# mdw771/adorym

Measured on AMD Instinct MI355X. Metric: probe-positions/sec (fwd+grad), 256^3 multislice ptycho, higher is better.
Workload: dtype f32

## Files before the change

adorym_amd/csrc/adm_object.hip:

```cpp
#include <hip/hip_runtime.h>
#include <cstdlib>
#include <cstring>
#include <hip/hip_fp16.h>
#include "adm_common.h"
#include "adm_optim.h"
#include "adm_ms_math.h"

namespace adm {

struct RotGeom {
    int Y, X, Z, Yp, Xp, pad_y0, pad_x0;
};

struct Bilin {
    int i00, i01, i10, i11;
    float w00, w01, w10, w11;
};

__device__ __forceinline__ Bilin make_bilin(const uint16_t* coords, int xr, int zr, int X, int Z) {
#pragma clang fp contract(off)
    Bilin b;
    if (coords == nullptr) {
        b.i00 = b.i01 = b.i10 = b.i11 = xr * Z + zr;
        b.w00 = 1.f; b.w01 = b.w10 = b.w11 = 0.f;
// ... 31 lines not shown
    const int ya = y_lo + blockIdx.z * y_chunk;
    const int yb = min(ya + y_chunk, y_hi);
    const size_t plane = (size_t)g.X * g.Z;
    for (int y = ya; y < yb; ++y) {
        const float2* o = obj + (size_t)y * plane;
        const float2 v00 = o[b.i00], v01 = o[b.i01], v10 = o[b.i10], v11 = o[b.i11];
        float2 r;
        r.x = v00.x * b.w00 + v01.x * b.w01 + v10.x * b.w10 + v11.x * b.w11;
        r.y = v00.y * b.w00 + v01.y * b.w01 + v10.y * b.w10 + v11.y * b.w11;
        const size_t o_rot = ((size_t)zr * g.Yp + g.pad_y0 + y) * g.Xp + g.pad_x0 + xr;
        if (rot) rot[o_rot] = r;
        if (trans) trans[o_rot] = slice_transmission(r, k1, sigma);
    }
}

__global__ __launch_bounds__(256) void rotate_fwd_stack_kernel(const float2* __restrict__ obj, const uint16_t* const* __restrict__ tables,
                                                               int Yb, float2* __restrict__ rot, float2* __restrict__ trans, float k1,
                                                               float sigma, RotGeom g, int y_chunk) {
    const int xr = blockIdx.x * 16 + (threadIdx.x & 15);
    const int zr = blockIdx.y * 16 + (threadIdx.x >> 4);
    if (xr >= g.X || zr >= g.Z) return;
    const int ya = blockIdx.z * y_chunk;
    const int r = ya / Yb;
    const Bilin b = make_bilin(tables[r], xr, zr, g.X, g.Z);
    const int yb = min(ya + y_chunk, g.Y);
    const size_t plane = (size_t)g.X * g.Z;
    for (int y = ya; y < yb; ++y) {
        const float2* o = obj + (size_t)(y - r * Yb) * plane;
        const float2 v00 = o[b.i00], v01 = o[b.i01], v10 = o[b.i10], v11 = o[b.i11];
        float2 q;
        q.x = v00.x * b.w00 + v01.x * b.w01 + v10.x * b.w10 + v11.x * b.w11;
        q.y = v00.y * b.w00 + v01.y * b.w01 + v10.y * b.w10 + v11.y * b.w11;
        const size_t o_rot = ((size_t)zr * g.Yp + g.pad_y0 + y) * g.Xp + g.pad_x0 + xr;
        if (rot) rot[o_rot] = q;
        if (trans) trans[o_rot] = slice_transmission(q, k1, sigma);
    }
}

__global__ __launch_bounds__(256) void identity_fwd_kernel(const float2* __restrict__ obj, float2* __restrict__ rot, float2* __restrict__ trans,
                                                           float k1, float sigma, RotGeom g, int y_lo, int y_hi) {
    const size_t n = (size_t)(y_hi - y_lo) * g.X * g.Z;
    for (size_t i = (size_t)blockIdx.x * blockDim.x + threadIdx.x; i < n; i += (size_t)gridDim.x * blockDim.x) {
        const int z = (int)(i % g.Z);
        const size_t yx = i / g.Z;
        const int x = (int)(yx % g.X), y = y_lo + (int)(yx / g.X);
        const float2 r = obj[((size_t)y * g.X + x) * g.Z + z];
        const size_t o_rot = ((size_t)z * g.Yp + g.pad_y0 + y) * g.Xp + g.pad_x0 + x;
        if (rot) rot[o_rot] = r;
        if (trans) trans[o_rot] = slice_transmission(r, k1, sigma);
    }
}
__global__ __launch_bounds__(256) void identity_adj_kernel(const float2* __restrict__ grot, float2* __restrict__ gobj, RotGeom g, int y_lo,
                                                           int y_hi) {
    const size_t n = (size_t)(y_hi - y_lo) * g.X * g.Z;
    for (size_t i = (size_t)blockIdx.x * blockDim.x + threadIdx.x; i < n; i += (size_t)gridDim.x * blockDim.x) {
        const int z = (int)(i % g.Z);
        const size_t yx = i / g.Z;
        const int x = (int)(yx % g.X), y = y_lo + (int)(yx / g.X);
        const float2 v = grot[((size_t)z * g.Yp + g.pad_y0 + y) * g.Xp + g.pad_x0 + x];
        float2* o = gobj + ((size_t)y * g.X + x) * g.Z + z;
        float2 c = *o;
        c.x += v.x;
        c.y += v.y;
        *o = c;
    }
}

__global__ __launch_bounds__(256) void transmission_kernel(const float2* __restrict__ rot, float2* __restrict__ trans, float k1,
                                                           float sigma, int Z, int Yp, int Xp, int row_lo, int row_hi) {
    const size_t per = (size_t)(row_hi - row_lo) * Xp;
    const size_t n = per * Z;
    for (size_t i = (size_t)blockIdx.x * blockDim.x + threadIdx.x; i < n; i += (size_t)gridDim.x * blockDim.x) {
        const size_t z = i / per, r = i - z * per;
        const size_t o = (z * Yp + row_lo) * Xp + r;
        trans[o] = rot ? slice_transmission(rot[o], k1, sigma) : make_float2(1.f, 0.f);
    }
}

__global__ __launch_bounds__(256) void rotate_adj_kernel(const float2* __restrict__ grot, const uint16_t* __restrict__ coords,
                                                         float* __restrict__ gobj, RotGeom g, int y_lo, int y_hi, int y_chunk) {
    const int xr = blockIdx.x * 16 + (threadIdx.x & 15);
    const int zr = blockIdx.y * 16 + (threadIdx.x >> 4);
    if (xr >= g.X || zr >= g.Z) return;
    const Bilin b = make_bilin(coords, xr, zr, g.X, g.Z);
    const int ya = y_lo + blockIdx.z * y_chunk;
    const int yb = min(ya + y_chunk, y_hi);
    const size_t plane = (size_t)g.X * g.Z;
    for (int y = ya; y < yb; ++y) {
        const float2 v = grot[((size_t)zr * g.Yp + g.pad_y0 + y) * g.Xp + g.pad_x0 + xr];
        float* o = gobj + 2 * (size_t)y * plane;
        if (b.w00 != 0.f) { atomicAdd(o + 2 * b.i00, v.x * b.w00); atomicAdd(o + 2 * b.i00 + 1, v.y * b.w00); }
        if (b.w01 != 0.f) { atomicAdd(o + 2 * b.i01, v.x * b.w01); atomicAdd(o + 2 * b.i01 + 1, v.y * b.w01); }
        if (b.w10 != 0.f) { atomicAdd(o + 2 * b.i10, v.x * b.w10); atomicAdd(o + 2 * b.i10 + 1, v.y * b.w10); }
        if (b.w11 != 0.f) { atomicAdd(o + 2 * b.i11, v.x * b.w11); atomicAdd(o + 2 * b.i11 + 1, v.y * b.w11); }
    }
}

template <bool ALONG_X>
__global__ __launch_bounds__(256) void rotate_adj_csr_kernel(const float2* __restrict__ grot, const int* __restrict__ ptr,
                                                             const int* __restrict__ src, const float* __restrict__ wgt,
                                                             float2* __restrict__ gobj, RotGeom g, int y_lo, int y_hi) {
    __shared__ float2 tile[4][16][17];
    const int lx = ALONG_X ? (threadIdx.x & 15) : (threadIdx.x >> 4);
    const int lz = ALONG_X ? (threadIdx.x >> 4) : (threadIdx.x & 15);
    const int x = blockIdx.x * 16 + lx, z = blockIdx.y * 16 + lz;
    const bool ok = (x < g.X) && (z < g.Z);
    const int t = ok ? x * g.Z + z : 0;
    const int beg = ok ? ptr[t] : 0, end = ok ? ptr[t + 1] : 0;
    const int y0 = y_lo + blockIdx.z * 4;
    const int ny = min(4, y_hi - y0);
    const size_t plane = (size_t)g.X * g.Z;
    float2 a[4];
#pragma unroll
    for (int i = 0; i < 4; ++i) a[i] = make_float2(0.f, 0.f);
    const size_t row = (size_t)(g.pad_y0 + y0) * g.Xp;
    if (ny == 4) {
        for (int j = beg; j < end; ++j) {
            const float w = wgt[j];
            const float2* q = grot + (size_t)src[j] + row;
            const float2 v0 = q[0], v1 = q[g.Xp], v2 = q[2 * (size_t)g.Xp], v3 = q[3 * (size_t)g.Xp];
            a[0].x += w * v0.x; a[0].y += w * v0.y;
            a[1].x += w * v1.x; a[1].y += w * v1.y;
            a[2].x += w * v2.x; a[2].y += w * v2.y;
            a[3].x += w * v3.x; a[3].y += w * v3.y;
        }
    } else {
        for (int j = beg; j < end; ++j) {
            const float w = wgt[j];
            const float2* q = grot + (size_t)src[j] + row;
#pragma unroll
            for (int i = 0; i < 4; ++i)
                if (i < ny) { const float2 v = q[(size_t)i * g.Xp]; a[i].x += w * v.x; a[i].y += w * v.y; }
        }
    }
    int wx = lx, wz = lz;
    if (ALONG_X) {
#pragma unroll
        for (int i = 0; i < 4; ++i) tile[i][lx][lz] = a[i];
        __syncthreads();
        wx = threadIdx.x >> 4; wz = threadIdx.x & 15;
#pragma unroll
        for (int i = 0; i < 4; ++i) a[i] = tile[i][wx][wz];
    }
    const int ox = blockIdx.x * 16 + wx, oz = blockIdx.y * 16 + wz;
    if (ox < g.X && oz < g.Z) {
        float2* o = gobj + (size_t)y0 * plane + (size_t)ox * g.Z + oz;
#pragma unroll
        for (int i = 0; i < 4; ++i)
            if (i < ny) { float2 c = o[(size_t)i * plane]; c.x += a[i].x; c.y += a[i].y; o[(size_t)i * plane] = c; }
    }
}

#define ADM_STAGE_MAX 1024
__global__ __launch_bounds__(256) void rotate_adj_staged_kernel(const float2* __restrict__ grot, const int* __restrict__ ptr,
                                                                const int* __restrict__ src, const unsigned short* __restrict__ lsrc,
                                                                const float* __restrict__ wgt,
                                                                const int4* __restrict__ boxes, float2* __restrict__ gobj, RotGeom g,
                                                                int y_lo, int y_hi) {
    __shared__ float2 stage[4 * ADM_STAGE_MAX];
    const int4 box = boxes[blockIdx.y * gridDim.x + blockIdx.x];
    const int y0 = y_lo + blockIdx.z * 4;
    const int ny = min(4, y_hi - y0);
    const int bw = box.z, bh = box.w, per = bw * bh;
    const size_t slice = (size_t)g.Yp * g.Xp;
    const size_t plane = (size_t)g.X * g.Z;
    const int lx = threadIdx.x >> 4, lz = threadIdx.x & 15;
    const int x = blockIdx.x * 16 + lx, z = blockIdx.y * 16 + lz;
    const bool ok = (x < g.X) && (z < g.Z);
    const int t = ok ? x * g.Z + z : 0;
    const int beg = ok ? ptr[t] : 0, end = ok ? ptr[t + 1] : 0;
    float2* o = gobj + (size_t)y0 * plane + (size_t)x * g.Z + z;
    if (bw == 0) {
        if (!ok) return;
        const size_t row = (size_t)(g.pad_y0 + y0) * g.Xp;
        float2 a[4];
#pragma unroll
        for (int i = 0; i < 4; ++i) a[i] = make_float2(0.f, 0.f);
        for (int j = beg; j < end; ++j) {
            const float w = wgt[j];
            const float2* q = grot + (size_t)src[j] + row;
#pragma unroll
            for (int i = 0; i < 4; ++i)
                if (i < ny) { const float2 v = q[(size_t)i * g.Xp]; a[i].x += w * v.x; a[i].y += w * v.y; }
        }
#pragma unroll
        for (int i = 0; i < 4; ++i)
            if (i < ny) { float2 c = o[(size_t)i * plane]; c.x += a[i].x; c.y += a[i].y; o[(size_t)i * plane] = c; }
        return;
    }
    if (per <= ADM_STAGE_MAX) {
        for (int idx = threadIdx.x; idx < 4 * per; idx += 256) {
            const int p = idx / per, rem = idx - p * per;
            const int zz = rem / bw, xx = rem - zz * bw;
            float2 v = make_float2(0.f, 0.f);
            if (p < ny) v = grot[(size_t)(box.y + zz) * slice + (size_t)(g.pad_y0 + y0 + p) * g.Xp + g.pad_x0 + box.x + xx];
            stage[p * ADM_STAGE_MAX + rem] = v;
        }
        __syncthreads();
        if (!ok) return;
        float2 a[4];
#pragma unroll
        for (int i = 0; i < 4; ++i) a[i] = make_float2(0.f, 0.f);
        for (int j = beg; j < end; ++j) {
            const float w = wgt[j];
            const int q = lsrc[j];
#pragma unroll
            for (int i = 0; i < 4; ++i) { const float2 v = stage[i * ADM_STAGE_MAX + q]; a[i].x += w * v.x; a[i].y += w * v.y; }
        }
#pragma unroll
        for (int i = 0; i < 4; ++i)
            if (i < ny) { float2 c = o[(size_t)i * plane]; c.x += a[i].x; c.y += a[i].y; o[(size_t)i * plane] = c; }
        return;
    }
    const int npp = (2 * per <= 4 * ADM_STAGE_MAX) ? 2 : 1;
    for (int p0 = 0; p0 < ny; p0 += npp) {
        for (int idx = threadIdx.x; idx < npp * per; idx += 256) {
            const int pp = idx / per, rem = idx - pp * per;
            const int zz = rem / bw, xx = rem - zz * bw;
            float2 v = make_float2(0.f, 0.f);
            if (p0 + pp < ny) v = grot[(size_t)(box.y + zz) * slice + (size_t)(g.pad_y0 + y0 + p0 + pp) * g.Xp + g.pad_x0 + box.x + xx];
            stage[idx] = v;
        }
        __syncthreads();
        if (ok) {
            float2 acc0 = make_float2(0.f, 0.f), acc1 = make_float2(0.f, 0.f);
            const int second = (npp == 2) ? per : 0;
            for (int j = beg; j < end; j += 8) {
                float w[8];
                int q[8];
#pragma unroll
                for (int u = 0; u < 8; ++u) {
                    const int jj = min(j + u, end - 1);
                    w[u] = (j + u < end) ? wgt[jj] : 0.f;
                    q[u] = lsrc[jj];
                }
#pragma unroll
                for (int u = 0; u < 8; ++u) {
                    const float2 v0 = stage[q[u]];
                    const float2 v1 = stage[q[u] + second];
                    acc0.x += w[u] * v0.x; acc0.y += w[u] * v0.y;
                    acc1.x += w[u] * v1.x; acc1.y += w[u] * v1.y;
                }
            }
            float2 c = o[(size_t)p0 * plane];
            c.x += acc0.x;
            c.y += acc0.y;
            o[(size_t)p0 * plane] = c;
            if (npp == 2 && p0 + 1 < ny) {
                float2 d = o[(size_t)(p0 + 1) * plane];
                d.x += acc1.x;
                d.y += acc1.y;
                o[(size_t)(p0 + 1) * plane] = d;
            }
        }
        __syncthreads();
    }
}

struct AdjTables { const int* ptr; const int* src; const unsigned short* lsrc; const float* wgt; const int4* boxes; };
__global__ __launch_bounds__(256) void rotate_adj_staged_stack_kernel(const float2* __restrict__ grot, const AdjTables* __restrict__ tabs,
                                                                      int R, int Yb, float2* __restrict__ gobj, RotGeom g, int npl,
                                                                      float2* __restrict__ part) {
    __shared__ float2 stage[4 * ADM_STAGE_MAX];
    const int nzg = (Yb + npl - 1) / npl;
    const int zg = part ? (int)blockIdx.z % nzg : (int)blockIdx.z;
    const int r_lo = part ? (int)blockIdx.z / nzg : 0, r_hi = part ? r_lo + 1 : R;
    const int y0 = zg * npl;
    const int ny = min(npl, Yb - y0);
    const size_t slice = (size_t)g.Yp * g.Xp;
    const size_t plane = (size_t)g.X * g.Z;
    const int lx = threadIdx.x >> 4, lz = threadIdx.x & 15;
    const int x = blockIdx.x * 16 + lx, z = blockIdx.y * 16 + lz;
    const bool ok = (x < g.X) && (z < g.Z);
    const int t = ok ? x * g.Z + z : 0;
    float2* o = (part ? part + (size_t)r_lo * Yb * plane : gobj) + (size_t)y0 * plane + (size_t)x * g.Z + z;
    float2 c[4];
#pragma unroll
    for (int i = 0; i < 4; ++i) c[i] = (ok && i < ny && !part) ? o[(size_t)i * plane] : make_float2(0.f, 0.f);
    for (int r = r_lo; r < r_hi; ++r) {
        const AdjTables T = tabs[r];
        const int4 box = T.boxes[blockIdx.y * gridDim.x + blockIdx.x];
        const int ys = r * Yb + y0;
        const int bw = box.z, bh = box.w, per = bw * bh;
        const int beg = ok ? T.ptr[t] : 0, end = ok ? T.ptr[t + 1] : 0;
        if (bw == 0) {
            const size_t row = (size_t)(g.pad_y0 + ys) * g.Xp;
            float2 a[4];
#pragma unroll
            for (int i = 0; i < 4; ++i) a[i] = make_float2(0.f, 0.f);
            for (int j = beg; j < end; ++j) {
                const float w = T.wgt[j];
                const float2* q = grot + (size_t)T.src[j] + row;
#pragma unroll
                for (int i = 0; i < 4; ++i)
                    if (i < ny) { const float2 v = q[(size_t)i * g.Xp]; a[i].x += w * v.x; a[i].y += w * v.y; }
            }
#pragma unroll
            for (int i = 0; i < 4; ++i) { c[i].x += a[i].x; c[i].y += a[i].y; }
        } else if (per <= ADM_STAGE_MAX) {
            for (int idx = threadIdx.x; idx < npl * per; idx += 256) {
                const int p = idx / per, rem = idx - p * per;
                const int zz = rem / bw, xx = rem - zz * bw;
                float2 v = make_float2(0.f, 0.f);
                if (p < ny) v = grot[(size_t)(box.y + zz) * slice + (size_t)(g.pad_y0 + ys + p) * g.Xp + g.pad_x0 + box.x + xx];
                stage[p * ADM_STAGE_MAX + rem] = v;
            }
            __syncthreads();
            float2 a[4];
#pragma unroll
            for (int i = 0; i < 4; ++i) a[i] = make_float2(0.f, 0.f);
            for (int j = beg; j < end; ++j) {
                const float w = T.wgt[j];
                const int q = T.lsrc[j];
#pragma unroll
                for (int i = 0; i < 4; ++i)
                    if (i < ny) { const float2 v = stage[i * ADM_STAGE_MAX + q]; a[i].x += w * v.x; a[i].y += w * v.y; }
            }
#pragma unroll
            for (int i = 0; i < 4; ++i) { c[i].x += a[i].x; c[i].y += a[i].y; }
        } else {
            const int npp = (npl >= 2 && 2 * per <= 4 * ADM_STAGE_MAX) ? 2 : 1;
            for (int p0 = 0; p0 < ny; p0 += npp) {
                for (int idx = threadIdx.x; idx < npp * per; idx += 256) {
                    const int pp = idx / per, rem = idx - pp * per;
                    const int zz = rem / bw, xx = rem - zz * bw;
                    float2 v = make_float2(0.f, 0.f);
                    if (p0 + pp < ny) v = grot[(size_t)(box.y + zz) * slice + (size_t)(g.pad_y0 + ys + p0 + pp) * g.Xp + g.pad_x0 + box.x + xx];
                    stage[idx] = v;
                }
                __syncthreads();
                float2 acc0 = make_float2(0.f, 0.f), acc1 = make_float2(0.f, 0.f);
                const int second = (npp == 2) ? per : 0;
                for (int j = beg; j < end; j += 8) {
                    float w[8];
                    int q[8];
#pragma unroll
                    for (int u = 0; u < 8; ++u) {
                        const int jj = min(j + u, end - 1);
                        w[u] = (j + u < end) ? T.wgt[jj] : 0.f;
                        q[u] = T.lsrc[jj];
                    }
#pragma unroll
                    for (int u = 0; u < 8; ++u) {
                        const float2 v0 = stage[q[u]];
                        const float2 v1 = stage[q[u] + second];
                        acc0.x += w[u] * v0.x; acc0.y += w[u] * v0.y;
                        acc1.x += w[u] * v1.x; acc1.y += w[u] * v1.y;
                    }
                }
#pragma unroll
                for (int i = 0; i < 4; ++i) {
                    if (i == p0) { c[i].x += acc0.x; c[i].y += acc0.y; }
                    if (npp == 2 && i == p0 + 1) { c[i].x += acc1.x; c[i].y += acc1.y; }
                }
                __syncthreads();
            }
        }
        __syncthreads();
    }
    if (ok) {
#pragma unroll
        for (int i = 0; i < 4; ++i)
            if (i < ny) o[(size_t)i * plane] = c[i];
    }
}

#define ADM_MAXCOVER 64

struct TileGeom {
    int Yp, Xp, pad_y0, pad_x0, Py, Px, R1, R2, G, LPW, NT, n_steps, binning, Z;
    int pixel_major;
    int row_elems;
    int row0, nrows;
    int add_lo, add_hi;
};

__global__ __launch_bounds__(256) void cover_build_kernel(const int2* __restrict__ pos, int b0, int B, TileGeom g,
                                                          unsigned* __restrict__ cover, int* __restrict__ overflow) {
    __shared__ int2 sp[256];
    __shared__ int sb[256];
    __shared__ int wcnt[4];
    const int x = blockIdx.x * 32 + (threadIdx.x & 31);
    const int r = blockIdx.y * 8 + (threadIdx.x >> 5);
    const bool live = x < g.Xp && r < g.nrows;
    const int y = g.row0 + r;
    const int bx_lo = blockIdx.x * 32, by_lo = g.row0 + blockIdx.y * 8;
    const size_t cplane = (size_t)g.nrows * g.Xp;
    unsigned* out = cover + (size_t)(live ? r : 0) * g.Xp + (live ? x : 0);
    int cnt = 0;
    const unsigned per_pos = (unsigned)g.n_steps * g.row_elems;
    const int wave = threadIdx.x >> 6, lane = threadIdx.x & 63;
    for (int c0 = b0; c0 < B; c0 += 256) {
        const int b = c0 + (int)threadIdx.x;
        int2 p = make_int2(0, 0);
        bool hit = false;
        if (b < B) {
            p = pos[b];
            const int ty = p.x + g.pad_y0, tx = p.y + g.pad_x0;
            hit = ty < by_lo + 8 && ty + g.Py > by_lo && tx < bx_lo + 32 && tx + g.Px > bx_lo;
        }
        const unsigned long long m = __ballot(hit);
        __syncthreads();
        if (lane == 0) wcnt[wave] = __popcll(m);
        __syncthreads();
        int off = 0, n = 0;
#pragma unroll
        for (int w = 0; w < 4; ++w) { if (w < wave) off += wcnt[w]; n += wcnt[w]; }
        if (hit) {
            const int k = off + __popcll(m & ((1ull << lane) - 1ull));
// ... 559 lines not shown
    if (reg_value) {
        __shared__ float red[4];
#pragma unroll
        for (int off = 32; off > 0; off >>= 1) val += __shfl_down(val, off, 64);
        if ((threadIdx.x & 63) == 0) red[threadIdx.x >> 6] = val;
        __syncthreads();
        if (threadIdx.x == 0) atomicAdd(reg_value, red[0] + red[1] + red[2] + red[3]);
    }
}

__global__ __launch_bounds__(256) void axpy_kernel(float* __restrict__ y, const float* __restrict__ x, float a, size_t n) {
    for (size_t i = (size_t)blockIdx.x * blockDim.x + threadIdx.x; i < n; i += (size_t)gridDim.x * blockDim.x)
        y[i] += a * x[i];
}

static inline int stream_grid(size_t n) {
    size_t b = (n + 255) / 256;
    return (int)(b > 4096 ? 4096 : (b ? b : 1));
}

}

using namespace adm;

extern "C" int adm_rotate_fwd(adm_plan* plan, const float* obj, const uint16_t* coords, float* obj_rot, int y_lo, int y_hi) {
    if (!plan || !obj || !obj_rot) return fail(ADM_ERR_INVALID, "adm_rotate_fwd: null argument");
    const adm_plan_desc& d = plan->d;
    if (y_lo < 0 || y_hi > d.obj_y || y_lo > y_hi) return fail(ADM_ERR_INVALID, "adm_rotate_fwd: bad y range");
    if (y_lo == y_hi) return ADM_OK;
    RotGeom g{d.obj_y, d.obj_x, d.obj_z, plan->Yp, plan->Xp, d.pad_y0, d.pad_x0};
    int y_chunk = 32;
    const int n_patch = ((d.obj_x + 15) / 16) * ((d.obj_z + 15) / 16);
    while (y_chunk > 1 && n_patch * ((y_hi - y_lo + y_chunk - 1) / y_chunk) < 512) y_chunk >>= 1;
    dim3 grid((d.obj_x + 15) / 16, (d.obj_z + 15) / 16, (y_hi - y_lo + y_chunk - 1) / y_chunk);
    float2* rot_out = (plan->trans_dev && plan->trans_only) ? (float2*)nullptr : (float2*)obj_rot;
    if (!coords && d.obj_z < 16)
        hipLaunchKernelGGL(identity_fwd_kernel, dim3(stream_grid((size_t)(y_hi - y_lo) * d.obj_x * d.obj_z)), dim3(256), 0, plan->ctx->stream,
                           (const float2*)obj, rot_out, plan->trans_dev, d.k1, (float)d.sign_convention, g, y_lo, y_hi);
    else
        hipLaunchKernelGGL(rotate_fwd_kernel, grid, dim3(256), 0, plan->ctx->stream, (const float2*)obj, coords, rot_out, plan->trans_dev,
                           d.k1, (float)d.sign_convention, g, y_lo, y_hi, y_chunk);
    ADM_HIP(hipGetLastError());
    if (plan->trans_dev) plan->trans_src = obj_rot;
    return ADM_OK;
}

extern "C" int adm_rotate_fwd_stack(adm_plan* plan, const float* obj, const void* tables_dev, int n_tables, float* obj_rot) {
    if (!plan || !obj || !tables_dev || !obj_rot) return fail(ADM_ERR_INVALID, "adm_rotate_fwd_stack: null argument");
    const adm_plan_desc& d = plan->d;
    if (n_tables < 1 || d.obj_y % n_tables) return fail(ADM_ERR_INVALID, "adm_rotate_fwd_stack: the plan's y extent is not n_tables blocks");
    const int Yb = d.obj_y / n_tables;
    RotGeom g{d.obj_y, d.obj_x, d.obj_z, plan->Yp, plan->Xp, d.pad_y0, d.pad_x0};
    int y_chunk = 32;
    while (y_chunk > 1 && Yb % y_chunk) y_chunk >>= 1;
    const int n_patch = ((d.obj_x + 15) / 16) * ((d.obj_z + 15) / 16);
    while (y_chunk > 1 && n_patch * (d.obj_y / y_chunk) < 512) y_chunk >>= 1;
    dim3 grid((d.obj_x + 15) / 16, (d.obj_z + 15) / 16, d.obj_y / y_chunk);
    float2* rot_out = (plan->trans_dev && plan->trans_only) ? (float2*)nullptr : (float2*)obj_rot;
    hipLaunchKernelGGL(rotate_fwd_stack_kernel, grid, dim3(256), 0, plan->ctx->stream, (const float2*)obj,
                       (const uint16_t* const*)tables_dev, Yb, rot_out, plan->trans_dev, d.k1, (float)d.sign_convention, g, y_chunk);
    ADM_HIP(hipGetLastError());
    if (plan->trans_dev) plan->trans_src = obj_rot;
    return ADM_OK;
}

static int transmission_fill(adm_plan* plan, const float* obj_rot, int row_lo, int row_hi) {
    const adm_plan_desc& d = plan->d;
    const size_t n = (size_t)(row_hi - row_lo) * plan->Xp * d.obj_z;
    hipLaunchKernelGGL(transmission_kernel, dim3((unsigned)std::min<size_t>((n + 255) / 256, 8192)), dim3(256), 0, plan->ctx->stream,
                       (const float2*)obj_rot, plan->trans_dev, d.k1, (float)d.sign_convention, d.obj_z, plan->Yp, plan->Xp, row_lo,
                       row_hi);
    ADM_HIP(hipGetLastError());
    return ADM_OK;
}

extern "C" int adm_plan_set_transmission_cache(adm_plan* plan, int on) {
    if (!plan) return fail(ADM_ERR_INVALID, "adm_plan_set_transmission_cache: null plan");
    const adm_plan_desc& d = plan->d;
    if (!on) {
        if (plan->trans_dev) {
            ADM_HIP(hipStreamSynchronize(plan->ctx->main_stream));
            ADM_HIP(hipFree(plan->trans_dev));
        }
        plan->trans_dev = nullptr;
        plan->trans_src = nullptr;
        plan->trans_only = false;
        return ADM_OK;
    }
    if (d.unknown_type != 0 || d.binning != 1)
        return fail(ADM_ERR_UNSUPPORTED, "adm_plan_set_transmission_cache: needs unknown_type delta_beta and binning 1");
    if (!plan->trans_dev) {
        float2* t = nullptr;
        ADM_HIP(hipMalloc((void**)&t, (size_t)d.obj_z * plan->Yp * plan->Xp * sizeof(float2)));
        plan->trans_dev = t;
        plan->trans_src = nullptr;
        const int rc = transmission_fill(plan, nullptr, 0, plan->Yp);
        if (rc) {
            (void)hipFree(t);
            plan->trans_dev = nullptr;
            plan->trans_only = false;
            return rc;
        }
    }
    plan->trans_only = (on == 2);
    return ADM_OK;
}

extern "C" int adm_transmission_refresh(adm_plan* plan, const float* obj_rot, int y_lo, int y_hi) {
    if (!plan || !obj_rot) return fail(ADM_ERR_INVALID, "adm_transmission_refresh: null argument");
    if (!plan->trans_dev) return fail(ADM_ERR_INVALID, "adm_transmission_refresh: the plan has no transmission cache");
    const adm_plan_desc& d = plan->d;
    if (y_lo < 0 || y_hi > d.obj_y || y_lo > y_hi) return fail(ADM_ERR_INVALID, "adm_transmission_refresh: bad y range");
    plan->trans_src = obj_rot;
    if (y_lo == y_hi) return ADM_OK;
    return transmission_fill(plan, obj_rot, d.pad_y0 + y_lo, d.pad_y0 + y_hi);
}

extern "C" int adm_rotate_adj(adm_plan* plan, const float* grad_rot, const uint16_t* coords, float* grad_obj, int y_lo, int y_hi) {
    if (!plan || !grad_rot || !grad_obj) return fail(ADM_ERR_INVALID, "adm_rotate_adj: null argument");
    const adm_plan_desc& d = plan->d;
    if (y_lo < 0 || y_hi > d.obj_y || y_lo > y_hi) return fail(ADM_ERR_INVALID, "adm_rotate_adj: bad y range");
    if (y_lo == y_hi) return ADM_OK;
    RotGeom g{d.obj_y, d.obj_x, d.obj_z, plan->Yp, plan->Xp, d.pad_y0, d.pad_x0};
    const int y_chunk = 32;
    dim3 grid((d.obj_x + 15) / 16, (d.obj_z + 15) / 16, (y_hi - y_lo + y_chunk - 1) / y_chunk);
    if (!coords && d.obj_z < 16)
        hipLaunchKernelGGL(identity_adj_kernel, dim3(stream_grid((size_t)(y_hi - y_lo) * d.obj_x * d.obj_z)), dim3(256), 0, plan->ctx->stream,
                           (const float2*)grad_rot, (float2*)grad_obj, g, y_lo, y_hi);
    else
        hipLaunchKernelGGL(rotate_adj_kernel, grid, dim3(256), 0, plan->ctx->stream, (const float2*)grad_rot, coords, grad_obj, g, y_lo,
                           y_hi, y_chunk);
    ADM_HIP(hipGetLastError());
    return ADM_OK;
}

extern "C" int adm_rotate_adj_csr(adm_plan* plan, const float* grad_rot, const int32_t* csr_ptr, const int32_t* csr_src,
                                  const float* csr_w, float* grad_obj, int y_lo, int y_hi, int lanes_along_x) {
    if (!plan || !grad_rot || !csr_ptr || !csr_src || !csr_w || !grad_obj) return fail(ADM_ERR_INVALID, "adm_rotate_adj_csr: null argument");
    const adm_plan_desc& d = plan->d;
    if (y_lo < 0 || y_hi > d.obj_y || y_lo > y_hi) return fail(ADM_ERR_INVALID, "adm_rotate_adj_csr: bad y range");
    if (y_lo == y_hi) return ADM_OK;
    RotGeom g{d.obj_y, d.obj_x, d.obj_z, plan->Yp, plan->Xp, d.pad_y0, d.pad_x0};
    dim3 grid((d.obj_x + 15) / 16, (d.obj_z + 15) / 16, (y_hi - y_lo + 3) / 4);
    if (lanes_along_x)
        hipLaunchKernelGGL(rotate_adj_csr_kernel<true>, grid, dim3(256), 0, plan->ctx->stream, (const float2*)grad_rot, csr_ptr, csr_src,
                           csr_w, (float2*)grad_obj, g, y_lo, y_hi);
    else
        hipLaunchKernelGGL(rotate_adj_csr_kernel<false>, grid, dim3(256), 0, plan->ctx->stream, (const float2*)grad_rot, csr_ptr, csr_src,
                           csr_w, (float2*)grad_obj, g, y_lo, y_hi);
    ADM_HIP(hipGetLastError());
    return ADM_OK;
}

extern "C" int adm_rotate_adj_staged(adm_plan* plan, const float* grad_rot, const int32_t* csr_ptr, const int32_t* csr_src,
                                     const uint16_t* csr_lsrc, const float* csr_w, const int32_t* boxes, float* grad_obj, int y_lo,
                                     int y_hi) {
    if (!plan || !grad_rot || !csr_ptr || !csr_src || !csr_lsrc || !csr_w || !boxes || !grad_obj)
        return fail(ADM_ERR_INVALID, "adm_rotate_adj_staged: null argument");
    const adm_plan_desc& d = plan->d;
    if (y_lo < 0 || y_hi > d.obj_y || y_lo > y_hi) return fail(ADM_ERR_INVALID, "adm_rotate_adj_staged: bad y range");
    if (y_lo == y_hi) return ADM_OK;
    RotGeom g{d.obj_y, d.obj_x, d.obj_z, plan->Yp, plan->Xp, d.pad_y0, d.pad_x0};
    dim3 grid((d.obj_x + 15) / 16, (d.obj_z + 15) / 16, (y_hi - y_lo + 3) / 4);
    hipLaunchKernelGGL(rotate_adj_staged_kernel, grid, dim3(256), 0, plan->ctx->stream, (const float2*)grad_rot, csr_ptr, csr_src,
                       (const unsigned short*)csr_lsrc, csr_w, (const int4*)boxes, (float2*)grad_obj, g, y_lo, y_hi);
    ADM_HIP(hipGetLastError());
    return ADM_OK;
}

#ifndef ADM_STACK_MIN_BLOCKS
#define ADM_STACK_MIN_BLOCKS 2048
#endif
__global__ __launch_bounds__(256) void stack_sum_kernel(const float2* __restrict__ part, int R, size_t n, float2* __restrict__ gobj) {
    const size_t i = (size_t)blockIdx.x * 256 + threadIdx.x;
    if (i >= n) return;
    float2 c = gobj[i];
    for (int r = 0; r < R; ++r) {
        const float2 a = part[(size_t)r * n + i];
        c.x += a.x;
        c.y += a.y;
    }
    gobj[i] = c;
}

extern "C" int adm_rotate_adj_staged_stack(adm_plan* plan, const float* grad_rot, const void* tables_dev, int n_tables, float* grad_obj,
                                           float* scratch, size_t scratch_bytes) {
    if (!plan || !grad_rot || !tables_dev || !grad_obj) return fail(ADM_ERR_INVALID, "adm_rotate_adj_staged_stack: null argument");
    const adm_plan_desc& d = plan->d;
    if (n_tables < 1 || d.obj_y % n_tables) return fail(ADM_ERR_INVALID, "adm_rotate_adj_staged_stack: the plan's y extent is not n_tables blocks");
    const int Yb = d.obj_y / n_tables;
    RotGeom g{d.obj_y, d.obj_x, d.obj_z, plan->Yp, plan->Xp, d.pad_y0, d.pad_x0};
    int npl = 4;
    const int n_patch = ((d.obj_x + 15) / 16) * ((d.obj_z + 15) / 16);
    while (npl > 1 && n_patch * ((Yb + npl - 1) / npl) < 1024) npl >>= 1;
    const size_t n_real = (size_t)Yb * d.obj_x * d.obj_z;
    if (scratch) {
        if (scratch_bytes < (size_t)n_tables * n_real * sizeof(float2))
            return fail(ADM_ERR_INVALID, "adm_rotate_adj_staged_stack: scratch smaller than n_tables x the real object");
        npl = 4;
        while (npl > 1 && (size_t)n_patch * ((Yb + npl - 1) / npl) * n_tables < (size_t)ADM_STACK_MIN_BLOCKS) npl >>= 1;
        dim3 gridp((d.obj_x + 15) / 16, (d.obj_z + 15) / 16, ((Yb + npl - 1) / npl) * n_tables);
        hipLaunchKernelGGL(rotate_adj_staged_stack_kernel, gridp, dim3(256), 0, plan->ctx->stream, (const float2*)grad_rot,
                           (const AdjTables*)tables_dev, n_tables, Yb, (float2*)grad_obj, g, npl, (float2*)scratch);
        hipLaunchKernelGGL(stack_sum_kernel, dim3((unsigned)((n_real + 255) / 256)), dim3(256), 0, plan->ctx->stream,
                           (const float2*)scratch, n_tables, n_real, (float2*)grad_obj);
        ADM_HIP(hipGetLastError());
        return ADM_OK;
    }
    dim3 grid((d.obj_x + 15) / 16, (d.obj_z + 15) / 16, (Yb + npl - 1) / npl);
    hipLaunchKernelGGL(rotate_adj_staged_stack_kernel, grid, dim3(256), 0, plan->ctx->stream, (const float2*)grad_rot,
                       (const AdjTables*)tables_dev, n_tables, Yb, (float2*)grad_obj, g, npl, (float2*)nullptr);
    ADM_HIP(hipGetLastError());
    return ADM_OK;
}

extern "C" int adm_tile_grad_accumulate(adm_plan* plan, void* workspace, size_t workspace_bytes, const int32_t* pos, int batch,
                                       const int32_t* pos_host, float* grad_rot) {
    return adm_tile_grad_accumulate_part(plan, workspace, workspace_bytes, pos, batch, pos_host, grad_rot, 0, 0, 0);
}

static int tile_geom(adm_plan* plan, int batch, const int32_t* pos_host, int win_y_lo, int win_y_hi, int add, TileGeom& g) {
    const adm_plan_desc& d = plan->d;
    const int N = d.probe_x;
    g.Yp = plan->Yp; g.Xp = plan->Xp; g.pad_y0 = d.pad_y0; g.pad_x0 = d.pad_x0; g.Py = d.probe_y; g.Px = d.probe_x;
    g.pixel_major = plan->generic ? 1 : 0;
    g.row_elems = (int)ms_row_elems(plan);
    g.R1 = g.R2 = g.G = g.LPW = 1; g.NT = 64;
    if (!plan->generic) { g.R1 = ms_r1_for(N); g.R2 = ms_r2_for(N); g.G = g.R1 > g.R2 ? g.R1 : g.R2; g.LPW = 64 / g.G; g.NT = ms_threads_for(N); }
    g.n_steps = plan->n_steps; g.binning = d.binning; g.Z = d.obj_z;
    int ymin = pos_host[0], ymax = pos_host[0];
    for (int b = 1; b < batch; ++b) { ymin = pos_host[2 * b] < ymin ? pos_host[2 * b] : ymin; ymax = pos_host[2 * b] > ymax ? pos_host[2 * b] : ymax; }
    g.row0 = ymin + d.pad_y0;
    g.nrows = ymax - ymin + d.probe_y;
    g.add_lo = g.add_hi = 0;
    if (add) {
        g.add_lo = g.row0;
        g.add_hi = g.row0 + g.nrows;
    } else if (win_y_hi > win_y_lo) {
        if (win_y_lo + d.pad_y0 > g.row0 || win_y_hi + d.pad_y0 < g.row0 + g.nrows)
            return fail(ADM_ERR_INVALID, "adm_tile_grad_accumulate_part: the window must contain the part's own rows");
        g.row0 = win_y_lo + d.pad_y0;
        g.nrows = win_y_hi - win_y_lo;
    }
    if (g.row0 < 0 || g.row0 + g.nrows > g.Yp) return fail(ADM_ERR_INVALID, "adm_tile_grad_accumulate: a position lies outside the padded frame");
    const size_t per = (size_t)plan->n_steps * g.row_elems;
    if ((size_t)batch * per >= 0xFFFFFFFFull) return fail(ADM_ERR_UNSUPPORTED, "adm_tile_grad_accumulate: batch too large for 32-bit tile offsets");
    return ADM_OK;
}

static unsigned long long pos_fingerprint(const int32_t* pos_host, int batch) {
    unsigned long long h = 1469598103934665603ull;
    for (int i = 0; i < 2 * batch; ++i) { h ^= (unsigned)pos_host[i]; h *= 1099511628211ull; }
    return h;
}
static void cover_key_put(adm_plan* plan, const void* ws, const void* pos, const int32_t* pos_host, int batch, const TileGeom& g) {
    int slot = 0;
    for (int i = 0; i < 4; ++i) {
        if (plan->cover_keys[i].ws == ws) { slot = i; break; }
        if (!plan->cover_keys[i].ws) slot = i;
    }
    plan->cover_keys[slot] = {ws, pos, batch, g.row0, g.nrows, pos_fingerprint(pos_host, batch)};
}
static bool cover_key_take(adm_plan* plan, const void* ws, const void* pos, const int32_t* pos_host, int batch, const TileGeom& g) {
    for (int i = 0; i < 4; ++i) {
        adm_plan::CoverKey& k = plan->cover_keys[i];
        if (k.ws == ws) {
            const bool ok = k.pos == pos && k.batch == batch && k.row0 == g.row0 && k.nrows == g.nrows && k.fp == pos_fingerprint(pos_host, batch);
            k.ws = nullptr;
            return ok;
        }
    }
    return false;
}

static int cover_build(adm_plan* plan, void* workspace, const int32_t* pos, int batch, const TileGeom& g, int b_lo = 0, int b_hi = -1) {
    if (b_hi < 0) b_hi = batch;
    char* ws = (char*)workspace;
    unsigned* cover = (unsigned*)(ws + ws_off_cover(plan, batch));
    int* overflow = (int*)(cover + (size_t)g.Yp * g.Xp * (ADM_MAXCOVER + 1));
    hipStream_t st = plan->ctx->stream;
    if (b_hi - b_lo > ADM_MAXCOVER) ADM_HIP(hipMemsetAsync(overflow, 0, sizeof(int), st));
    dim3 grid((g.Xp + 31) / 32, (g.nrows + 7) / 8, 1);
    hipLaunchKernelGGL(cover_build_kernel, grid, dim3(256), 0, st, (const int2*)pos, b_lo, b_hi, g, cover, overflow);
    ADM_HIP(hipGetLastError());
    return ADM_OK;
}

extern "C" int adm_tile_cover_build(adm_plan* plan, void* workspace, size_t workspace_bytes, const int32_t* pos, int batch,
                                    const int32_t* pos_host, int win_y_lo, int win_y_hi, int add) {
    if (!plan || !workspace || !pos || !pos_host) return fail(ADM_ERR_INVALID, "adm_tile_cover_build: null argument");
    if (batch <= 0) return fail(ADM_ERR_INVALID, "adm_tile_cover_build: batch must be positive");
    if (workspace_bytes < adm_plan_workspace_bytes(plan, batch)) return fail(ADM_ERR_INVALID, "adm_tile_cover_build: workspace too small");
    TileGeom g;
    int rc = tile_geom(plan, batch, pos_host, win_y_lo, win_y_hi, add, g);
    if (rc) return rc;
    rc = cover_build(plan, workspace, pos, batch, g);
    if (rc) return rc;
    cover_key_put(plan, workspace, pos, pos_host, batch, g);
    return ADM_OK;
}

extern "C" int adm_tile_grad_accumulate_part(adm_plan* plan, void* workspace, size_t workspace_bytes, const int32_t* pos, int batch,
                                            const int32_t* pos_host, float* grad_rot, int win_y_lo, int win_y_hi, int add) {
    if (!plan || !workspace || !pos || !pos_host || !grad_rot) return fail(ADM_ERR_INVALID, "adm_tile_grad_accumulate: null argument");
    if (batch <= 0) return fail(ADM_ERR_INVALID, "adm_tile_grad_accumulate: batch must be positive");
    if (workspace_bytes < adm_plan_workspace_bytes(plan, batch)) return fail(ADM_ERR_INVALID, "adm_tile_grad_accumulate: workspace too small");
    TileGeom g;
    int rc = tile_geom(plan, batch, pos_host, win_y_lo, win_y_hi, add, g);
    if (rc) return rc;
    const bool prebuilt = cover_key_take(plan, workspace, pos, pos_host, batch, g);
    if (!prebuilt) {
        rc = cover_build(plan, workspace, pos, batch, g);
        if (rc) return rc;
    }
    char* ws = (char*)workspace;
    const float2* gtile = (const float2*)(ws + ws_off_gtile(plan, batch));
    unsigned* cover = (unsigned*)(ws + ws_off_cover(plan, batch));
    hipStream_t st = plan->ctx->stream;
// ... 236 lines not shown
```

Before: 15110.

## Remap staged rotate-adjoint grid to 1D with per-plane border tiles and XCD-aware interior

The staged rotate-adjoint kernel now launches a flat 1D grid by default. Border-ring tiles that use the unstaged or large-box path are split into one block per y-plane to spread their heavier work, and interior tiles are distributed in contiguous chunks per XCD slot (block index mod 8) for better L2 locality across MI355X's chiplets. The old 3D grid remains available via ADM_ROT_XCD=0. The change adds index arithmetic and some early-exit padding blocks, and it assumes an 8-way round-robin dispatch of blocks to XCDs.

```diff
diff --git a/adorym_amd/csrc/adm_object.hip b/adorym_amd/csrc/adm_object.hip
--- a/adorym_amd/csrc/adm_object.hip
+++ b/adorym_amd/csrc/adm_object.hip
@@ -207,20 +207,15 @@
 }
 
 #define ADM_STAGE_MAX 1024
-__global__ __launch_bounds__(256) void rotate_adj_staged_kernel(const float2* __restrict__ grot, const int* __restrict__ ptr,
-                                                                const int* __restrict__ src, const unsigned short* __restrict__ lsrc,
-                                                                const float* __restrict__ wgt,
-                                                                const int4* __restrict__ boxes, float2* __restrict__ gobj, RotGeom g,
-                                                                int y_lo, int y_hi) {
-    __shared__ float2 stage[4 * ADM_STAGE_MAX];
-    const int4 box = boxes[blockIdx.y * gridDim.x + blockIdx.x];
-    const int y0 = y_lo + blockIdx.z * 4;
-    const int ny = min(4, y_hi - y0);
+__device__ __forceinline__ void adj_staged_planes(float2* __restrict__ stage, const float2* __restrict__ grot, const int* __restrict__ ptr,
+                                                  const int* __restrict__ src, const unsigned short* __restrict__ lsrc,
+                                                  const float* __restrict__ wgt, const int4 box, float2* __restrict__ gobj,
+                                                  const RotGeom& g, int bx, int bz, int y0, int ny) {
     const int bw = box.z, bh = box.w, per = bw * bh;
     const size_t slice = (size_t)g.Yp * g.Xp;
     const size_t plane = (size_t)g.X * g.Z;
     const int lx = threadIdx.x >> 4, lz = threadIdx.x & 15;
-    const int x = blockIdx.x * 16 + lx, z = blockIdx.y * 16 + lz;
+    const int x = bx * 16 + lx, z = bz * 16 + lz;
     const bool ok = (x < g.X) && (z < g.Z);
     const int t = ok ? x * g.Z + z : 0;
     const int beg = ok ? ptr[t] : 0, end = ok ? ptr[t + 1] : 0;
@@ -267,7 +262,7 @@
             if (i < ny) { float2 c = o[(size_t)i * plane]; c.x += a[i].x; c.y += a[i].y; o[(size_t)i * plane] = c; }
         return;
     }
-    const int npp = (2 * per <= 4 * ADM_STAGE_MAX) ? 2 : 1;
+    const int npp = (ny >= 2 && 2 * per <= 4 * ADM_STAGE_MAX) ? 2 : 1;
     for (int p0 = 0; p0 < ny; p0 += npp) {
         for (int idx = threadIdx.x; idx < npp * per; idx += 256) {
             const int pp = idx / per, rem = idx - pp * per;
@@ -310,6 +305,57 @@
         }
         __syncthreads();
     }
+}
+
+__global__ __launch_bounds__(256) void rotate_adj_staged_kernel(const float2* __restrict__ grot, const int* __restrict__ ptr,
+                                                                const int* __restrict__ src, const unsigned short* __restrict__ lsrc,
+                                                                const float* __restrict__ wgt,
+                                                                const int4* __restrict__ boxes, float2* __restrict__ gobj, RotGeom g,
+                                                                int y_lo, int y_hi, int xcd) {
+    __shared__ float2 stage[4 * ADM_STAGE_MAX];
+    const int nbx = (g.X + 15) / 16, nbz = (g.Z + 15) / 16;
+    if (!xcd) {
+        const int y0 = y_lo + blockIdx.z * 4;
+        adj_staged_planes(stage, grot, ptr, src, lsrc, wgt, boxes[blockIdx.y * nbx + blockIdx.x], gobj, g, blockIdx.x, blockIdx.y, y0,
+                          min(4, y_hi - y0));
+        return;
+    }
+    const int nyt = y_hi - y_lo;
+    const int rows = nbz > 1 ? 2 : 1, cols = nbx > 1 ? 2 : 1;
+    const int n_ring = rows * nbx + cols * max(nbz - 2, 0);
+    const int n_a = n_ring * nyt, n_a8 = (n_a + 7) & ~7;
+    const int b = blockIdx.x;
+    if (b < n_a) {
+        int e = b % n_ring, bx, bz;
+        const int yi = b / n_ring;
+        if (e < rows * nbx) {
+            bx = e % nbx;
+            bz = (e < nbx) ? 0 : nbz - 1;
+        } else {
+            e -= rows * nbx;
+            bx = (e % cols) ? nbx - 1 : 0;
+            bz = 1 + e / cols;
+        }
+        const int4 box = boxes[bz * nbx + bx];
+        int ny = 1;
+        if (box.z != 0 && box.z * box.w <= ADM_STAGE_MAX) {
+            if (yi & 3) return;
+            ny = min(4, nyt - yi);
+        }
+        adj_staged_planes(stage, grot, ptr, src, lsrc, wgt, box, gobj, g, bx, bz, y_lo + yi, ny);
+        return;
+    }
+    if (b < n_a8) return;
+    const int ix = nbx - 2, iz = nbz - 2;
+    if (ix <= 0 || iz <= 0) return;
+    const int n = ix * iz * ((nyt + 3) / 4), q = n >> 3, r = n & 7;
+    const int k = (b - n_a8) & 7, slot = (b - n_a8) >> 3;
+    if (slot >= q + (k < r)) return;
+    const int L = k * q + min(k, r) + slot;
+    const int gz = L / (ix * iz), pz = L - gz * ix * iz;
+    const int bz = 1 + pz / ix, bx = 1 + pz % ix;
+    const int y0 = y_lo + gz * 4;
+    adj_staged_planes(stage, grot, ptr, src, lsrc, wgt, boxes[bz * nbx + bx], gobj, g, bx, bz, y0, min(4, y_hi - y0));
 }
 
 struct AdjTables { const int* ptr; const int* src; const unsigned short* lsrc; const float* wgt; const int4* boxes; };
@@ -1175,6 +1221,11 @@
     return ADM_OK;
 }
 
+static bool rot_xcd_grid() {
+    const char* e = std::getenv("ADM_ROT_XCD");
+    return !(e && std::strcmp(e, "0") == 0);
+}
+
 extern "C" int adm_rotate_adj_staged(adm_plan* plan, const float* grad_rot, const int32_t* csr_ptr, const int32_t* csr_src,
                                      const uint16_t* csr_lsrc, const float* csr_w, const int32_t* boxes, float* grad_obj, int y_lo,
                                      int y_hi) {
@@ -1185,8 +1236,13 @@
     if (y_lo == y_hi) return ADM_OK;
     RotGeom g{d.obj_y, d.obj_x, d.obj_z, plan->Yp, plan->Xp, d.pad_y0, d.pad_x0};
     dim3 grid((d.obj_x + 15) / 16, (d.obj_z + 15) / 16, (y_hi - y_lo + 3) / 4);
-    hipLaunchKernelGGL(rotate_adj_staged_kernel, grid, dim3(256), 0, plan->ctx->stream, (const float2*)grad_rot, csr_ptr, csr_src,
-                       (const unsigned short*)csr_lsrc, csr_w, (const int4*)boxes, (float2*)grad_obj, g, y_lo, y_hi);
+    const bool xcd = rot_xcd_grid();
+    const int nbx = (int)grid.x, nbz = (int)grid.y;
+    const int n_ring = (nbz > 1 ? 2 : 1) * nbx + (nbx > 1 ? 2 : 1) * std::max(nbz - 2, 0);
+    const unsigned n = 8 * ((n_ring * (y_hi - y_lo) + 7) / 8) + 8 * ((std::max(nbx - 2, 0) * std::max(nbz - 2, 0) * (int)grid.z + 7) / 8);
+    hipLaunchKernelGGL(rotate_adj_staged_kernel, xcd ? dim3(n) : grid, dim3(256), 0, plan->ctx->stream, (const float2*)grad_rot,
+                       csr_ptr, csr_src, (const unsigned short*)csr_lsrc, csr_w, (const int4*)boxes, (float2*)grad_obj, g, y_lo, y_hi,
+                       (int)xcd);
     ADM_HIP(hipGetLastError());
     return ADM_OK;
 }
```

Result: faster. 15630 (median of 6 runs) (+3.5%).
